# IllyaArtemchuk/Harmonies-Alphazero

Measured on AMD Instinct MI355X. Metric: self-play env-steps/sec + games/sec @4096 boards, 1/2/4/8 GPUs; bit-exact vs CPU, higher is better.
Workload: dtype u64; 1 GPU; config2: 4096 concurrent boards/GPU, reset + rule-driven play to game end (legal mask, step, chance draws, final scoring); one step = 256 hz_play launches of 4096 boards; boards_per_gpu=4096, parallelism=shard1

## Files before the change

harmonies-alphazero_amd/csrc/hz_device.hpp:

```cpp
#pragma once
#include <hip/hip_runtime.h>
#include <stdint.h>

namespace hz {

constexpr int kCells = 23;
constexpr uint32_t kAll23 = (1u << 23) - 1;
constexpr int kActions = 143;
enum { WATER = 0, PLANT = 1, WOOD = 2, STONE = 3, BUILDING = 4, FIELD = 5 };
enum { PH_CHOOSE = 0, PH_P1 = 1, PH_P2 = 2, PH_P3 = 3, PH_OVER = 4 };
enum {
  ST_OK = 0, ST_BAD_PILE = 1, ST_BAD_FORMAT = 2, ST_NOT_IN_HAND = 3, ST_ILLEGAL_STACK = 4,
  ST_BAD_PHASE = 5, ST_BAD_ACTION = 6, ST_NOOP = 7
};

__host__ __device__ constexpr int initial_count(int t) {
  return t == WATER ? 23 : t == PLANT ? 19 : t == WOOD ? 21 : t == STONE ? 23 : t == BUILDING ? 15 : 19;
}

struct State {
  uint64_t pl[4];
  uint64_t piles;
  uint64_t misc;
};

__device__ __forceinline__ int hand_tile(uint64_t m, int j) { return (int)((m >> (3 * j)) & 7); }
__device__ __forceinline__ int hand_n(uint64_t m) { return (int)((m >> 9) & 3); }
__device__ __forceinline__ int bag_n(uint64_t m, int t) { return (int)((m >> (11 + 5 * t)) & 31); }
__device__ __forceinline__ int player_of(uint64_t m) { return (int)((m >> 41) & 1); }
__device__ __forceinline__ int phase_of(uint64_t m) { return (int)((m >> 42) & 7); }
__device__ __forceinline__ int over_flag(uint64_t m) { return (int)((m >> 45) & 1); }
__device__ __forceinline__ int winner_code(uint64_t m) { return (int)((m >> 46) & 3); }
__device__ __forceinline__ int score_of(uint64_t m, int p) { return (int)((m >> (48 + 8 * p)) & 255); }
__device__ __forceinline__ int npiles_of(uint64_t piles) { return (int)((piles >> 45) & 7); }
__device__ __forceinline__ int pile_tile(uint64_t piles, int i, int j) { return (int)((piles >> (9 * i + 3 * j)) & 7); }
// ... 323 lines not shown
    if (pos >= kMT) { pos = 0; tw = 0; }
    while (tw < kMT && tw < pos + W) tw += twist_block_vec(w, tw);
    left = tw - pos < W ? tw - pos : W;
    const int a = pos & ~3, sh = pos & 3;
    uint32_t f[W + 4];
#pragma unroll
    for (int k = 0; k < W / 4 + 1; k++) {
      const int o = a + 4 * k <= kMT - 4 ? a + 4 * k : kMT - 4;
      const uint4 v = *(const uint4*)(w + o);
      f[4 * k] = v.x; f[4 * k + 1] = v.y; f[4 * k + 2] = v.z; f[4 * k + 3] = v.w;
    }
#pragma unroll
    for (int j = 0; j < W; j++) q[j] = sh == 0 ? f[j] : sh == 1 ? f[j + 1] : sh == 2 ? f[j + 2] : f[j + 3];
  }

  __device__ __forceinline__ uint32_t next() {
    fresh = false;
    if (left > 0) {
      const uint32_t v = q[0];
#pragma unroll
      for (int j = 0; j + 1 < W; j++) q[j] = q[j + 1];
      left--;
      pos++;
      return temper(v);
    }
    if (pos >= kMT) { pos = 0; tw = 0; }
    if (pos >= tw) tw += twist_block(w, 1, tw);
    return temper(w[pos++]);
  }
};
using WinMT12 = WinGMT<12>;

constexpr int kLdsStride = 65;
extern __shared__ uint32_t hz_lds[];

struct LdsMT {
  int lane, pos, tw;
  __device__ __forceinline__ LdsMT(int l, int cursor) : lane(l), pos(cursor & 0xFFFF), tw(cursor >> 16) {}
  __device__ __forceinline__ int cursor() const { return pos | (tw << 16); }
  __device__ __forceinline__ uint32_t* w() const { return hz_lds + lane; }

  __device__ __forceinline__ void prefetch() {
    if (pos >= kMT) { pos = 0; tw = 0; }
    while (tw < kMT && tw < pos + 24) tw += twist_block(w(), kLdsStride, tw);
  }

  __device__ __forceinline__ uint32_t word(int i) const {
    return temper(hz_lds[(i < kMT ? i : kMT - 1) * kLdsStride + lane]);
  }

  __device__ __forceinline__ uint32_t next() {
    if (pos >= kMT) { pos = 0; tw = 0; }
    if (pos >= tw) tw += twist_block(w(), kLdsStride, tw);
    return word(pos++);
  }

  __device__ __forceinline__ void normalize() {
    if (pos >= kMT) return;
    while (tw < kMT) tw += twist_block(w(), kLdsStride, tw);
  }

  __device__ __forceinline__ void twist_ahead(int target) {
    if (pos >= kMT) { pos = 0; tw = 0; }
    while (tw < target) tw += twist_block(w(), kLdsStride, tw);
  }
};

constexpr int kAheadTwist = 224;
constexpr int kMTAhead = 0 | (kAheadTwist << 16);

struct InitGen { uint32_t v[kMT]; };
constexpr InitGen make_init_gen() {
  InitGen g{};
  uint32_t x = 19650218u;
  g.v[0] = x;
  for (int i = 1; i < kMT; i++) {
    x = 1812433253u * (x ^ (x >> 30)) + (uint32_t)i;
    g.v[i] = x;
  }
  return g;
}
__constant__ InitGen kInitGen = make_init_gen();

struct NoProgress {
  __device__ __forceinline__ void operator()(int) const {}
};
template <class Ptr, class Prog = NoProgress>
__device__ __forceinline__ void mt_seed(Ptr w, int stride, uint64_t seed, Prog prog = Prog()) {
  uint32_t key0 = (uint32_t)seed, key1 = (uint32_t)(seed >> 32);
  uint32_t kA = key0, kB = key1 ? key1 + 1u : key0;
  uint32_t prev = 19650218u;
  uint32_t iv[8];
#pragma unroll
  for (int u = 0; u < 8; u++) iv[u] = kInitGen.v[1 + u];
  for (int g = 1; g < kMT - 7; g += 8) {
    uint32_t nx[8];
#pragma unroll
    for (int u = 0; u < 8; u++) nx[u] = kInitGen.v[g + 8 + u < kMT ? g + 8 + u : kMT - 1];
#pragma unroll
    for (int u = 0; u < 8; u++) {
      uint32_t v = (iv[u] ^ ((prev ^ (prev >> 30)) * 1664525U)) + ((u & 1) ? kB : kA);
      w[(g + u) * stride] = v;
      prev = v;
    }
#pragma unroll
    for (int u = 0; u < 8; u++) iv[u] = nx[u];
  }
#pragma unroll
  for (int u = 0; u < 7; u++) {
    uint32_t v = (iv[u] ^ ((prev ^ (prev >> 30)) * 1664525U)) + ((u & 1) ? kB : kA);
    w[(617 + u) * stride] = v;
    prev = v;
  }
  uint32_t m1 = w[1 * stride];
// ... 171 lines not shown

template <class M>
__device__ __forceinline__ uint32_t randbelow(M& m, uint32_t n) {
  if (!n) return 0;
  int k = 32 - __clz(n);
  uint32_t r = m.next() >> (32 - k);
  while (r >= n) r = m.next() >> (32 - k);
  return r;
}

template <class M>
__device__ __forceinline__ void sample3_serial(M& m, uint32_t n, int k, uint32_t j[3], int got) {
  if (n <= 21) {
    for (int i = got; i < k; i++) j[i] = randbelow(m, n - (uint32_t)i);
  } else {
    for (int i = got; i < k; i++) {
      uint32_t v;
      bool dup;
      do {
        v = randbelow(m, n);
        dup = (i > 0 && j[0] == v) || (i > 1 && j[1] == v);
      } while (dup);
      j[i] = v;
    }
  }
}

template <class M>
__device__ __forceinline__ void sample3_raw(M& m, uint32_t n, int k, uint32_t j[3]) {
  sample3_serial(m, n, k, j, 0);
}

typedef __attribute__((address_space(3))) const volatile uint32_t LdsVolatileWord;
template <bool Clamp>
__device__ __forceinline__ uint32_t scan_word(const LdsMT& m, int t) {
  LdsVolatileWord* lds = (LdsVolatileWord*)hz_lds;
  if (Clamp) {
    int i = m.pos + t < kMT ? m.pos + t : kMT - 1;
    return lds[i * kLdsStride + m.lane];
  }
  return lds[(m.pos + t) * kLdsStride + m.lane];
}

__device__ __forceinline__ uint32_t sgpr_const(uint32_t v) {
  uint32_t r;
  asm volatile("s_mov_b32 %0, %1" : "=s"(r) : "i"(v));
  return r;
}
struct TemperMasks {
  uint32_t b, c;
  __device__ __forceinline__ TemperMasks() : b(sgpr_const(0x9d2c5680u)), c(sgpr_const(0xefc60000u)) {}
};
__device__ __forceinline__ uint32_t and_xor(uint32_t x, uint32_t m, uint32_t y) {
  uint32_t r;
  asm("v_bitop3_b32 %0, %1, %2, %3 bitop3:0x6a" : "=v"(r) : "v"(x), "s"(m), "v"(y));
  return r;
}
__device__ __forceinline__ uint32_t temper_top14(uint32_t y, const TemperMasks& k) {
  y ^= y >> 11;
  y = and_xor(y << 7, k.b, y);
  y = and_xor(y << 15, k.c, y);
  return y;
}
__device__ __forceinline__ uint32_t temper_top14(uint32_t y) {
  y ^= y >> 11;
  y ^= (y << 7) & 0x9d2c5680u;
  y ^= (y << 15) & 0xefc60000u;
  return y;
}

template <bool Clamp, bool Pool>
__device__ __forceinline__ int scan3(LdsMT& m, uint32_t n, uint32_t& p0, uint32_t& p1, uint32_t& p2) {
  int avail = m.tw - m.pos;
  uint32_t lim = n;
  int sh = __clz(n);
  uint32_t j0 = 0xffffffffu, j1 = 0xffffffffu, j2 = 0xffffffffu;
  int got = 0, used = 0;
  TemperMasks tk;
  uint32_t w[4], nx[4];
#pragma unroll
  for (int u = 0; u < 4; u++) nx[u] = scan_word<Clamp>(m, u);
#pragma unroll
  for (int seg = 0; seg < 6; seg++) {
#pragma unroll
    for (int u = 0; u < 4; u++) w[u] = nx[u];
    if (seg < 5) {
#pragma unroll
      for (int u = 0; u < 4; u++) nx[u] = scan_word<Clamp>(m, 4 * seg + 4 + u);
    }
#pragma unroll
    for (int u = 0; u < 4; u++) {
      int t = 4 * seg + u;
      bool live = got < 3;
      if (Clamp) live = live && t < avail;
      uint32_t v = temper_top14(w[u], tk) >> sh;
      bool ok = live && v < lim;
      if (!Pool) ok = ok && v != j0 && v != j1;
      j2 = ok ? j1 : j2;
      j1 = ok ? j0 : j1;
      j0 = ok ? v : j0;
      got += ok ? 1 : 0;
      used += live ? 1 : 0;
      if (Pool) {
        lim -= ok ? 1u : 0u;
        sh = __clz(lim);
      }
    }
    if (__all(got >= 3)) break;
  }
  m.pos += used;
  p0 = got == 3 ? j2 : got == 2 ? j1 : j0;
  p1 = got == 3 ? j1 : j0;
  p2 = j0;
  return got;
}

__device__ __forceinline__ void sample3_raw(LdsMT& m, uint32_t n, int k, uint32_t j[3]) {
  if (k != 3) {
    sample3_serial(m, n, k, j, 0);
    return;
  }
  uint32_t j0, j1, j2;
  int got;
  bool far = __any(m.pos > kMT - 24);
  if (__all(n > 21)) {
    if (far) got = scan3<true, false>(m, n, j0, j1, j2);
    else got = scan3<false, false>(m, n, j0, j1, j2);
  } else if (__all(n <= 21)) {
    if (far) got = scan3<true, true>(m, n, j0, j1, j2);
    else got = scan3<false, true>(m, n, j0, j1, j2);
  } else {
    if (n > 21) got = scan3<true, false>(m, n, j0, j1, j2);
    else got = scan3<true, true>(m, n, j0, j1, j2);
  }
  j[0] = j0; j[1] = j1; j[2] = j2;
  if (got < k) sample3_serial(m, n, k, j, got);
}

struct WinMT : LdsMT {
  int lim;
  __device__ __forceinline__ WinMT(int l, int cursor, int rows) : LdsMT(l, cursor), lim(rows) {}
  __device__ __forceinline__ void prefetch() {}
  __device__ __forceinline__ uint32_t next() {
    const int i = pos++;
    return i < lim ? temper(hz_lds[i * kLdsStride + lane]) : 0x9E3779B9u * (uint32_t)(i + 1);
  }
};
__device__ __forceinline__ void sample3_raw(WinMT& m, uint32_t n, int k, uint32_t j[3]) {
  if (k != 3) {
    sample3_serial(m, n, k, j, 0);
    return;
  }
  uint32_t j0, j1, j2;
  int got;
  LdsMT& lm = m;
  if (__all(n > 21)) got = scan3<false, false>(lm, n, j0, j1, j2);
  else if (__all(n <= 21)) got = scan3<false, true>(lm, n, j0, j1, j2);
  else if (n > 21) got = scan3<false, false>(lm, n, j0, j1, j2);
  else got = scan3<false, true>(lm, n, j0, j1, j2);
  j[0] = j0; j[1] = j1; j[2] = j2;
  if (got < k) sample3_serial(m, n, k, j, got);
}

template <class M>
__device__ __forceinline__ int draw_pile(uint64_t misc, M& m, uint32_t& pile9) {
  int cnt[6];
#pragma unroll
  for (int t = 0; t < 6; t++) cnt[t] = bag_n(misc, t);
  uint32_t n = 0;
#pragma unroll
  for (int t = 0; t < 6; t++) n += (uint32_t)cnt[t];
  pile9 = 0x1FF;
  if (!n) return 0;
  int k = n < 3 ? (int)n : 3;
  uint32_t j[3] = {0, 0, 0};
  sample3_raw(m, n, k, j);
  uint32_t idx[3];
  if (n <= 21) {
    uint32_t mp0 = 0xffffffffu, mp1 = 0xffffffffu, mv0 = 0, mv1 = 0;
#pragma unroll
    for (int i = 0; i < 3; i++) {
      uint32_t ji = j[i], last = n - (uint32_t)i - 1;
      uint32_t vj = ji, vl = last;
      if (i > 0 && mp0 == ji) vj = mv0;
      if (i > 1 && mp1 == ji) vj = mv1;
      if (i > 0 && mp0 == last) vl = mv0;
      if (i > 1 && mp1 == last) vl = mv1;
      idx[i] = vj;
      if (i == 0) { mp0 = ji; mv0 = vl; }
      if (i == 1) { mp1 = ji; mv1 = vl; }
    }
  } else {
// ... 645 lines not shown
```

harmonies-alphazero_amd/csrc/hz_env.hip:

```cpp
#include <hip/hip_runtime.h>

#include <cstdio>
#include <cstdlib>
#include <cstring>

#include "../../include/hz_abi.h"
#include "hz_device.hpp"
#include "hz_encode.hpp"
#include "hz_host.hpp"

using namespace hz;
using namespace hz_host;

struct P2Draw {
  int32_t *tag;
  int32_t *k;
  uint64_t *q;
  uint64_t *bag;
  int32_t *c;
};
struct P2Mid {
  int32_t *tag;
  uint64_t *st;
  uint64_t *q;
// ... 1244 lines not shown
    ply[b] = g_ply;
    seed[b] = sd;
#if defined(HZ_DIAG) && !defined(HZ_DIAG_ROLES_ONLY)
    if (g_stamps) {
      uint64_t *o = g_stamps + (size_t)b * 16;
      o[8] = acc8; o[9] = acc9; o[10] = acc10; o[11] = acc11; o[12] = acc12; o[13] = acc13;
    }
#endif
    if (games_done) games_done[b] = games;
    if (steps_done) steps_done[b] = steps;
    if (ep_final) ep_final[b] = episode[b];
    uint64_t lm = __ballot(lds_used);
    if (lane == 0) s_lds_mask = lm;
  }
  if (w0 && !act && lane == 0 && actmask == 0) s_lds_mask = 0;
  __syncthreads();
  uint64_t lds_mask = s_lds_mask & actmask;
  if (lds_mask) stage_mt(g, nb, tid, lds_mask, false);
#ifdef HZ_DIAG
  if (g_stamps && threadIdx.x < 64 && act) g_stamps[(size_t)b * 16 + 5] = __builtin_amdgcn_s_memtime() - role_t0;
#endif
}

#ifndef HZ_P2_ST_WT
#define HZ_P2_ST_WT 0
#endif
#ifndef HZ_P2_AUX
#define HZ_P2_AUX 16
#endif
constexpr int kP2Win = 96;
constexpr int kP2WinRows = kP2Win + 24;
#ifndef HZ_P2_DCUT
#if HZ_P2_NDRAW == 5
#define HZ_P2_DCUT 0, 5, 10, 14, 18
#elif HZ_P2_NDRAW == 4
#define HZ_P2_DCUT 0, 7, 13, 18
#endif
#endif
constexpr int kP2DCut[kP2Draw] = {HZ_P2_DCUT};
constexpr int kP2StageDraws = 7;
#ifndef HZ_P2_PCUT
#if HZ_P2_NPLAY == 5
#define HZ_P2_PCUT 16, 32, 48, 64
#elif HZ_P2_NPLAY == 4
#define HZ_P2_PCUT 24, 40, 56
#endif
#endif
constexpr int kP2PCut[kP2Play - 1] = {HZ_P2_PCUT};
enum { kWvP1 = 8, kWvHash = 9, kWvPlay = 10, kWvIdle = 15 };
#ifndef HZ_P2_WAVES
#if HZ_P2_NDRAW == 5 && HZ_P2_NPLAY == 5
#define HZ_P2_WAVES 0, 1, 4, 9, 2, 3, 8, 10
#elif HZ_P2_NDRAW == 5
#define HZ_P2_WAVES 0, 1, 4, 9, 2, 3, 8, 15
#elif HZ_P2_NPLAY == 5
#define HZ_P2_WAVES 0, 1, 8, 9, 2, 3, 10, 15
#else
#define HZ_P2_WAVES 0, 1, 8, 9, 2, 3, 15, 15
#endif
#endif
constexpr int kP2Wave[8] = {HZ_P2_WAVES};
constexpr int p2_wave_count(int code) {
  int c = 0;
  for (int k = 0; k < 8; k++) c += kP2Wave[k] == code;
  return c;
}
constexpr bool p2_waves_ok() {
  for (int d = 0; d < 5; d++)
    if (p2_wave_count(d) != (d < kP2Draw ? 1 : 0)) return false;
  return p2_wave_count(kWvP1) == 1 && p2_wave_count(kWvHash) == 1 && p2_wave_count(kWvPlay) == (kP2Play == 5 ? 1 : 0);
}
static_assert(p2_waves_ok(), "HZ_P2_WAVES: every stage outside the seed and play blocks on exactly one wave");
constexpr int kP2MinPlies = 96;
#ifdef HZ_DIAG
constexpr int kP2Stamps = 48;
#define P2_PHASE(slot, t0)                                                                                       \
  do {                                                                                                           \
    __builtin_amdgcn_sched_barrier(0);                                                                           \
    if (g_stamps && b < a.n) g_stamps[(size_t)b * kP2Stamps + (slot)] = __builtin_amdgcn_s_memtime() - (t0); \
    __builtin_amdgcn_sched_barrier(0);                                                                           \
  } while (0)
#else
#define P2_PHASE(slot, t0) \
  do {                     \
  } while (0)
#endif
static_assert(4 * kP2WinRows * kLdsStride * 4 <= (int)kResetLds, "a window per wave of a draw block");

struct P2Args {
  uint64_t *st;
  uint32_t *mt;
  int32_t *pos, *ply, *episode;
  uint64_t *seed;
  int n, max_plies, draws;
  int cut[kP2Play - 1];
  int dcut[kP2Draw + 1];
  uint64_t seed_base;
  long nrow;
  int32_t *games_done, *steps_done, *mt_src;
  const int32_t *ep_in;
  int32_t *ep_out;
  uint32_t *s_mt[kP2Stages];
  int32_t *s_tag[kP2Stages];
  int32_t *s_cur[kP2Stages];
  int s_idx_last;
  uint32_t *p1h_w;
  const uint32_t *p1h_r;
  int32_t *p1t_w;
  const int32_t *p1t_r;
  uint32_t *p2h_w;
  const uint32_t *p2h_r;
  uint32_t *p3h_w;
  const uint32_t *p3h_r;
  P2Draw x_w[kP2Draw - 1], x_r[kP2Draw - 1];
  P2Draw pl_w, pl_r[kP2Play];
  P2Mid m_w[kP2Play - 1], m_r[kP2Play - 1];
  uint32_t *h_w;
  const uint32_t *h_r[kP2Play];
  int32_t *ht_w;
  const int32_t *ht_r[kP2Play];
// ... 121 lines not shown
    v = kMT + 1;
  }
  return v;
}
__device__ __forceinline__ void p2_publish(int *flag, int v) {
  asm volatile("" ::: "memory");
  __hip_atomic_store(flag, v, __ATOMIC_RELAXED, __HIP_MEMORY_SCOPE_WORKGROUP);
}
__device__ __forceinline__ __amdgpu_buffer_rsrc_t p2_slot_rsrc(uint32_t *slot, int b0, size_t nr) {
  const uint64_t base = (uint64_t)(slot + b0);
  uint32_t lo = __builtin_amdgcn_readfirstlane((uint32_t)base), hi = __builtin_amdgcn_readfirstlane((uint32_t)(base >> 32));
  const int bytes = __builtin_amdgcn_readfirstlane((int)((size_t)kMT * nr * 4 - (size_t)b0 * 4));
  return __builtin_amdgcn_make_buffer_rsrc((void *)(((uint64_t)hi << 32) | lo), 0, bytes, 0x00020000);
}
#ifndef HZ_P2_LDNT
#define HZ_P2_LDNT 0
#endif
__device__ __forceinline__ uint4 p2_ld4(const uint32_t *p) {
  if constexpr (HZ_P2_LDNT) {
    typedef uint32_t v4u __attribute__((ext_vector_type(4)));
    const v4u v = __builtin_nontemporal_load((const v4u *)p);
    return make_uint4(v[0], v[1], v[2], v[3]);
  }
  return *reinterpret_cast<const uint4 *>(p);
}
template <class T>
__device__ __forceinline__ void p2_st(T *p, T v) {
  if constexpr (HZ_P2_AUX == 16 && HZ_P2_ST_WT) __hip_atomic_store(p, v, __ATOMIC_RELAXED, __HIP_MEMORY_SCOPE_AGENT);
  else *p = v;
}
__device__ __forceinline__ uint32_t p1_step(uint32_t t, uint32_t q, bool odd, uint32_t kA, uint32_t kB) {
  return (t ^ ((q ^ (q >> 30)) * 1664525U)) + (odd ? kA : kB);
}
__device__ __forceinline__ int p2_tab(int i) { return i < kMT ? i : kMT - 1; }
__device__ __forceinline__ uint32_t p1_row1(uint32_t kA, uint32_t kB) {
  return p1_step(kInitGen.v[1], 19650218u, true, kA, kB);
}
__device__ __forceinline__ void p2_keys(uint64_t seed, uint32_t &kA, uint32_t &kB) {
  const uint32_t key0 = (uint32_t)seed, key1 = (uint32_t)(seed >> 32);
  kA = key0;
  kB = key1 ? key1 + 1u : key0;
}

__device__ __forceinline__ void p2_p1(const P2Args &a, int b) {
  const int e = a.ep_in[b] + kP2Last;
  uint32_t kA, kB;
  p2_keys(episode_seed(a.seed_base, b, e), kA, kB);
  uint32_t prev = 19650218u;
  uint32_t iv[8];
#pragma unroll
  for (int u = 0; u < 8; u++) iv[u] = kInitGen.v[1 + u];
#pragma unroll 1
  for (int g = 1; g < 617; g += 8) {
    uint32_t nx[8];
#pragma unroll
    for (int u = 0; u < 8; u++) nx[u] = kInitGen.v[p2_tab(g + 8 + u)];
    __builtin_amdgcn_sched_barrier(0);
#pragma unroll
    for (int u = 0; u < 8; u++) prev = p1_step(iv[u], prev, !(u & 1), kA, kB);
    __builtin_amdgcn_sched_barrier(0);
#pragma unroll
    for (int u = 0; u < 8; u++) iv[u] = nx[u];
  }
#pragma unroll
  for (int u = 0; u < 7; u++) prev = p1_step(iv[u], prev, !(u & 1), kA, kB);
  a.p1h_w[b] = p1_step(p1_row1(kA, kB), prev, false, kA, kB);
  a.p1t_w[b] = e * 8 + 2;
}

constexpr int kP2aEnd = 209, kP2bEnd = 417;
constexpr int kTwKeep = 397;
struct P2Ahead {
  uint32_t cur[8];
  uint32_t iv[8];
  uint32_t last;
};
template <int G>
__device__ __forceinline__ void p2_ahead_init(P2Ahead &h, uint32_t q, uint32_t kA, uint32_t kB) {
#pragma unroll
  for (int u = 0; u < 8; u++) {
    q = p1_step(kInitGen.v[p2_tab(G + u)], q, (G + u) & 1, kA, kB);
    h.cur[u] = q;
  }
#pragma unroll
  for (int u = 0; u < 8; u++) h.iv[u] = kInitGen.v[p2_tab(G + 8 + u)];
  h.last = q;
}
__device__ __forceinline__ uint32_t twist_part(uint32_t cur, uint32_t next) {
  const uint32_t y = (cur & 0x80000000U) | (next & 0x7fffffffU);
  return (y >> 1) ^ ((y & 1U) ? 0x9908b0dfU : 0U);
}
enum { kP2Final = 0, kP2Keep = 1, kP2Part = 2 };
template <int G0, int G1, int Mode>
__device__ __forceinline__ void p2_span(int lane, __amdgpu_buffer_rsrc_t rs, int row_bytes, uint32_t &prev, P2Ahead &h,
                                        uint32_t kA, uint32_t kB, int *prog) {
  constexpr bool KeepLds = Mode == kP2Keep;
  static_assert((G1 - G0) % 8 == 0, "groups of eight");
  uint32_t *l = hz_lds + lane;
  constexpr int S = kLdsStride;
#pragma unroll 2
  for (int g = G0; g < G1; g += 8) {
    uint32_t ivn[8], nx[8];
#pragma unroll
    for (int u = 0; u < 8; u++) ivn[u] = kInitGen.v[p2_tab(g + 16 + u)];
    const uint32_t kneg = __builtin_amdgcn_readfirstlane(0u - (uint32_t)g);
    const int soff = __builtin_amdgcn_readfirstlane((Mode == kP2Part ? g - 1 : g) * row_bytes);
    uint32_t q = h.cur[7];
#pragma unroll
    for (int u = 0; u < 8; u++) {
      const uint32_t p = (prev ^ (prev >> 30)) * 1566083941U;
      uint32_t v;
      asm("v_xad_u32 %0, %1, %2, %3" : "=v"(v) : "v"(p), "v"(h.cur[u]), "s"(kneg - (uint32_t)u));
      __builtin_amdgcn_raw_buffer_store_b32(Mode == kP2Part ? twist_part(prev, v) : v, rs, lane * 4,
                                            soff + u * row_bytes, HZ_P2_AUX);
      if (KeepLds) l[(g + u) * S] = v;
      prev = v;
      q = p1_step(h.iv[u], q, (G0 + u) & 1, kA, kB);
      nx[u] = q;
    }
    if (KeepLds) p2_publish(prog, g + 8);
    h.last = h.cur[7];
#pragma unroll
    for (int u = 0; u < 8; u++) {
      h.cur[u] = nx[u];
      h.iv[u] = ivn[u];
    }
  }
}
template <int G, int G1, int Mode>
__device__ __forceinline__ void p2_tail(int lane, __amdgpu_buffer_rsrc_t rs, int row_bytes, uint32_t &prev, P2Ahead &h) {
  static_assert(G1 - G >= 1 && G1 - G <= 8, "within the group ahead");
#pragma unroll
  for (int i = G; i < G1; i++) {
    const uint32_t v = (h.cur[i - G] ^ ((prev ^ (prev >> 30)) * 1566083941U)) - (uint32_t)i;
    if (Mode == kP2Part) __builtin_amdgcn_raw_buffer_store_b32(twist_part(prev, v), rs, lane * 4, (i - 1) * row_bytes, HZ_P2_AUX);
    else __builtin_amdgcn_raw_buffer_store_b32(v, rs, lane * 4, i * row_bytes, HZ_P2_AUX);
    if (Mode == kP2Keep) hz_lds[i * kLdsStride + lane] = v;
    prev = v;
  }
  h.last = h.cur[G1 - G - 1];
}

template <int K>
__device__ __forceinline__ void p2_third(const P2Args &a, int b0, int lane, int e, bool ok, int *s_prog) {
  const int b = b0 + lane;
  const bool act = b < a.n;
  const size_t nr = (size_t)a.nrow;
  if (K == 0 && act && !ok) a.s_tag[1][b] = -1;
  if (!__any(ok)) {
    if (K == 2) p2_publish(s_prog, kMT + 1);
    return;
  }
  uint32_t *slot = a.s_mt[1 + K];
  uint32_t kA, kB;
  p2_keys(episode_seed(a.seed_base, b, e), kA, kB);
  uint32_t prev, first1, row2, q;
  if (K == 0) {
    first1 = act ? a.p1h_r[b] : 0u;
    prev = first1;
    q = p1_row1(kA, kB);
  } else {
    const uint32_t *h = K == 1 ? a.p2h_r : a.p3h_r;
    prev = act ? h[b] : 0u;
    first1 = act ? h[nr + b] : 0u;
    row2 = act ? h[2 * nr + b] : 0u;
    q = act ? h[3 * nr + b] : 0u;
  }
  const __amdgpu_buffer_rsrc_t rs = p2_slot_rsrc(slot, b0, nr);
  const int row_bytes = (int)(nr * 4);
  P2Ahead h;
  if constexpr (K == 0) {
    q = p1_step(kInitGen.v[2], q, false, kA, kB);
    row2 = (q ^ ((prev ^ (prev >> 30)) * 1566083941U)) - 2U;
    prev = row2;
    p2_ahead_init<3>(h, q, kA, kB);
    constexpr int G = 3 + 8 * ((kP2aEnd - 3) / 8);
    p2_span<3, G, kP2Part>(lane, rs, row_bytes, prev, h, kA, kB, s_prog);
    p2_tail<G, kP2aEnd, kP2Part>(lane, rs, row_bytes, prev, h);
  } else if constexpr (K == 1) {
    static_assert(kAheadTwist + 1 - kP2aEnd == 16, "P2b's part steps: two groups");
    p2_ahead_init<kP2aEnd>(h, q, kA, kB);
    p2_span<kP2aEnd, kAheadTwist + 1, kP2Part>(lane, rs, row_bytes, prev, h, kA, kB, s_prog);
    __builtin_amdgcn_raw_buffer_store_b32(prev, rs, lane * 4, kAheadTwist * row_bytes, HZ_P2_AUX);
    p2_span<kAheadTwist + 1, kP2bEnd, kP2Final>(lane, rs, row_bytes, prev, h, kA, kB, s_prog);
  } else {
    const uint32_t f0 = act ? slot[(size_t)397 * nr + b] : 0u, f1 = act ? slot[(size_t)398 * nr + b] : 0u;
    p2_ahead_init<kP2bEnd>(h, q, kA, kB);
    constexpr int G = kP2bEnd + 8 * ((kMT - kP2bEnd) / 8);
    p2_span<kP2bEnd, G, kP2Keep>(lane, rs, row_bytes, prev, h, kA, kB, s_prog);
    p2_tail<G, kMT, kP2Keep>(lane, rs, row_bytes, prev, h);
    p2_publish(s_prog, kMT);
    const uint32_t row1 = (first1 ^ ((prev ^ (prev >> 30)) * 1566083941U)) - 1U;
    __builtin_amdgcn_raw_buffer_store_b32(f0 ^ twist_part(0x80000000u, row1), rs, lane * 4, 0, HZ_P2_AUX);
    __builtin_amdgcn_raw_buffer_store_b32(f1 ^ twist_part(row1, row2), rs, lane * 4, row_bytes, HZ_P2_AUX);
  }
  if (K < 2) {
    if (ok) {
      uint32_t *ho = K == 0 ? a.p2h_w : a.p3h_w;
      ho[b] = prev;
      ho[nr + b] = first1;
      ho[2 * nr + b] = row2;
      ho[3 * nr + b] = h.last;
      a.s_tag[1 + K][b] = e * 8 + 3 + K;
    }
  } else if (ok) {
    a.s_tag[3][b] = e * 8 + 5;
  }
}

constexpr int kTwIters = kAheadTwist / 4;
constexpr int kTwHbm = (kP2bEnd - 397 + 3) / 4;
__device__ __forceinline__ uint4 xor4(const uint4 &a, const uint4 &b) {
  return make_uint4(a.x ^ b.x, a.y ^ b.y, a.z ^ b.z, a.w ^ b.w);
}
__device__ __forceinline__ void p2_twist(const P2Args &a, int b0, int lane, bool any, int *s_prog) {
  if (!any) return;
  const size_t nr = (size_t)a.nrow;
  uint32_t *slot = a.s_mt[3];
  const int grp = lane >> 4, c4 = (lane & 15) * 4;
  uint32_t *col = slot + b0 + c4;
  auto row = [&](int r) { return p2_ld4(col + (size_t)r * nr); };
  const __amdgpu_buffer_rsrc_t rs = p2_slot_rsrc(slot, b0, nr);
  const int row_bytes = __builtin_amdgcn_readfirstlane((int)(nr * 4));
// ... 43 lines not shown
  const bool act = b < a.n;
  if (tid == 0) s_prog = 0;
  const int k = w < 3 ? w : 2;
  const int e = act ? a.ep_in[b] + kP2Last - 1 - k : 0;
  const bool ok = act && (k == 0 ? a.p1t_r[b] : a.s_tag[1 + k][b]) == e * 8 + 2 + k;
  __syncthreads();
  if (w == 0) p2_third<0>(a, b0, lane, e, ok, &s_prog);
  else if (w == 1) p2_third<1>(a, b0, lane, e, ok, &s_prog);
  else if (w == 2) p2_third<2>(a, b0, lane, e, ok, &s_prog);
  else p2_twist(a, b0, lane, __any(ok), &s_prog);
}

__device__ __forceinline__ int wave_min_i(int v) {
#pragma unroll
  for (int o = 32; o > 0; o >>= 1) v = min(v, __shfl_xor(v, o));
  return v;
}
__device__ __forceinline__ void p2_draw_stage(const P2Args &a, int b0, int lane, int stage, int base) {
  const int b = b0 + lane;
#ifdef HZ_DIAG
  const uint64_t t0 = __builtin_amdgcn_s_memtime();
#endif
  const bool act = b < a.n;
  const size_t nr = (size_t)a.nrow;
  const int d0 = a.dcut[stage], d1 = stage == kP2Draw - 1 ? a.draws : min(a.draws, a.dcut[stage + 1]);
  const int e = act ? a.ep_in[b] + kP2Last - kP2SDraw - stage : 0;
  const uint32_t *slot = a.s_mt[kP2SDraw + stage];
  int32_t *cur = a.s_cur[kP2SDraw + stage] + b;
  const P2Draw &in = a.x_r[stage > 0 ? stage - 1 : 0];
  const P2Draw &out = stage == kP2Draw - 1 ? a.pl_w : a.x_w[stage < kP2Draw - 1 ? stage : 0];
  bool ok = act && a.s_tag[kP2SDraw + stage][b] == e * 8 + 5;
  int k0 = 0, c0 = kMTAhead;
  uint64_t bag = initial_bag(), q[kAheadWords] = {0, 0, 0, 0};
  if (stage > 0 && act) {
    const int itag = in.tag[b];
    k0 = in.k[b];
    c0 = in.c[b];
    bag = in.bag[b];
#pragma unroll
    for (int i = 0; i < kAheadWords; i++) q[i] = in.q[(size_t)i * nr + b];
    ok = ok && itag == e * 8 + stage;
  }
  const bool draws = ok && k0 >= d0 && d0 < d1;
  const int r0 = wave_min_i(draws ? (c0 & 0xFFFF) : kAheadTwist) & ~3;
  if (r0 < kAheadTwist) {
    constexpr int U = kP2Win / 4;
    const int c4 = (lane & 15) * 4;
    uint4 v[U];
#pragma unroll
    for (int u = 0; u < U; u++) {
      const int r = r0 + 4 * u + (lane >> 4);
      v[u] = p2_ld4(slot + (size_t)r * nr + b0 + c4);
    }
#pragma unroll
    for (int u = 0; u < U; u++) {
      uint32_t *dd = hz_lds + base + (4 * u + (lane >> 4)) * kLdsStride + c4;
      dd[0] = v[u].x;
      dd[1] = v[u].y;
      dd[2] = v[u].z;
      dd[3] = v[u].w;
    }
  }
  P2_PHASE(28 + stage, t0);
  if (!act) return;
  if (!ok) {
    out.tag[b] = -1;
    return;
  }
  if (stage == 0) cur[0] = kMTAhead;
  int k = k0, cc = c0;
  if (draws) {
    const int lim = min(r0 + kP2Win, kAheadTwist);
    StreamDraw<WinMT> d{WinMT(base - r0 * kLdsStride + lane, c0, lim)};
#pragma unroll 1
    for (int i = d0; i < d1; i++) {
      if (d.m.pos >= lim) break;
      const uint32_t p9 = d(bag);
      if (d.m.pos > lim) break;
      apply_pile_fast(bag, p9);
      const int bit = 9 * i, wd = bit >> 6, off = bit & 63;
      const uint64_t lo9 = (uint64_t)p9 << off, hi9 = off > 55 ? (uint64_t)p9 >> (64 - off) : 0ull;
      q[0] |= wd == 0 ? lo9 : 0ull;
      q[1] |= wd == 1 ? lo9 : wd == 0 ? hi9 : 0ull;
      q[2] |= wd == 2 ? lo9 : wd == 1 ? hi9 : 0ull;
      q[3] |= wd == 3 ? lo9 : wd == 2 ? hi9 : 0ull;
      cc = d.m.cursor();
      p2_st(&cur[(size_t)(i + 1) * nr], cc);
      k = i + 1;
    }
  }
  p2_st(&out.k[b], k);
  p2_st(&out.c[b], cc);
  p2_st(&out.bag[b], bag);
#pragma unroll
  for (int i = 0; i < kAheadWords; i++) p2_st(&out.q[(size_t)i * nr + b], q[i]);
  p2_st(&out.tag[b], e * 8 + stage + 1);
}

__device__ __forceinline__ void p2_hashes(const P2Args &a, int b) {
  const size_t nr = (size_t)a.nrow;
  const int e = a.ep_in[b] + kP2Last - (kP2SPlay - 1);
  const uint64_t rk = rule_key(episode_seed(a.seed_base, b, e));
#pragma unroll 1
  for (int j = 0; j < kRulePlies; j++) p2_st(&a.h_w[(size_t)j * nr + b], rule_h32(rk, j));
  a.ht_w[b] = e;
}

__device__ __forceinline__ void p2_draw(const P2Args &a, int blk, int code) {
  const int tid = threadIdx.x, lane = tid & 63, w = tid >> 6;
  const int b0 = blk * kBlock;
  if (code < kP2Draw) {
    p2_draw_stage(a, b0, lane, code, w * kP2WinRows * kLdsStride);
  } else if (code == kWvP1 && b0 + lane < a.n) {
    p2_p1(a, b0 + lane);
  } else if (code == kWvHash && b0 + lane < a.n) {
    p2_hashes(a, b0 + lane);
  }
}

__device__ __forceinline__ void p2_mid_put(const P2Mid &m, size_t nr, int b, const State &s, const PlayDraw2 &d, int g,
                                           int e) {
#pragma unroll
  for (int k = 0; k < 4; k++) p2_st(&m.st[(size_t)k * nr + b], s.pl[k]);
  p2_st(&m.st[4 * nr + b], s.piles);
  p2_st(&m.st[5 * nr + b], s.misc);
  p2_st(&m.q[b], d.q0);
  p2_st(&m.q[nr + b], d.q1);
  p2_st(&m.q[2 * nr + b], d.q2);
  p2_st(&m.q[3 * nr + b], d.q3);
  p2_st(&m.i[b], d.d);
  p2_st(&m.i[nr + b], g);
  p2_st(&m.i[2 * nr + b], d.fell ? d.gm.cursor() : -1);
  p2_st(&m.tag[b], e);
}
__device__ __forceinline__ PlayDraw2 p2_mid_get(const P2Mid &m, size_t nr, int b, State &s, int &g, int nd,
                                               uint32_t *slot, const int32_t *cur) {
#pragma unroll
  for (int k = 0; k < 4; k++) s.pl[k] = m.st[(size_t)k * nr + b];
  s.piles = m.st[4 * nr + b];
  s.misc = m.st[5 * nr + b];
  const int d = m.i[b], fc = m.i[2 * nr + b];
  g = m.i[nr + b];
  return PlayDraw2{m.q[b], m.q[nr + b], m.q[2 * nr + b], m.q[3 * nr + b], d, nd, fc >= 0,
                   MTR(slot, (int)nr, fc >= 0 ? fc : 0), cur + (size_t)nd * nr};
}
// ... 781 lines not shown
```

Before: 21.66 billion env-steps/s.

## Vectorize MT init-table scalar loads, pad LDS window stride, rebalance draw stages

Pads the constant MT init table so row 1 sits on a 64-byte boundary and the read-ahead needs no clamping. The P1 seeding loop can then use double-buffered s_load_dwordx8 scalar loads, and the P2 spans read the table through a constant-address-space pointer. The draw window in LDS gets a stride of 68 so rows are 16-byte aligned and can be written with uint4 stores. Stage 0 issues its window load before reading the previous stage's inputs. It also moves the P2b/P2c split point and the draw-stage cut points, and uses v_bfi in twist_part. The risks are scalar-load hazards from the inline asm, a larger LDS footprint and retuned stage balance.

```diff
diff --git a/harmonies-alphazero_amd/csrc/hz_device.hpp b/harmonies-alphazero_amd/csrc/hz_device.hpp
--- a/harmonies-alphazero_amd/csrc/hz_device.hpp
+++ b/harmonies-alphazero_amd/csrc/hz_device.hpp
@@ -1,6 +1,8 @@
 #pragma once
 #include <hip/hip_runtime.h>
 #include <stdint.h>
+
+#include "hz_initgen.hpp"
 
 namespace hz {
 
@@ -390,7 +392,7 @@
 using WinMT12 = WinGMT<12>;
 
 constexpr int kLdsStride = 65;
-extern __shared__ uint32_t hz_lds[];
+extern __shared__ __attribute__((aligned(16))) uint32_t hz_lds[];
 
 struct LdsMT {
   int lane, pos, tw;
@@ -427,17 +429,7 @@
 constexpr int kAheadTwist = 224;
 constexpr int kMTAhead = 0 | (kAheadTwist << 16);
 
-struct InitGen { uint32_t v[kMT]; };
-constexpr InitGen make_init_gen() {
-  InitGen g{};
-  uint32_t x = 19650218u;
-  g.v[0] = x;
-  for (int i = 1; i < kMT; i++) {
-    x = 1812433253u * (x ^ (x >> 30)) + (uint32_t)i;
-    g.v[i] = x;
-  }
-  return g;
-}
+static_assert(kInitGenRows == kMT, "the table's rows");
 __constant__ InitGen kInitGen = make_init_gen();
 
 struct NoProgress {
@@ -675,14 +667,14 @@
 }
 
 typedef __attribute__((address_space(3))) const volatile uint32_t LdsVolatileWord;
-template <bool Clamp>
+template <bool Clamp, int Stride = kLdsStride>
 __device__ __forceinline__ uint32_t scan_word(const LdsMT& m, int t) {
   LdsVolatileWord* lds = (LdsVolatileWord*)hz_lds;
   if (Clamp) {
     int i = m.pos + t < kMT ? m.pos + t : kMT - 1;
-    return lds[i * kLdsStride + m.lane];
-  }
-  return lds[(m.pos + t) * kLdsStride + m.lane];
+    return lds[i * Stride + m.lane];
+  }
+  return lds[(m.pos + t) * Stride + m.lane];
 }
 
 __device__ __forceinline__ uint32_t sgpr_const(uint32_t v) {
@@ -712,7 +704,7 @@
   return y;
 }
 
-template <bool Clamp, bool Pool>
+template <bool Clamp, bool Pool, int Stride = kLdsStride>
 __device__ __forceinline__ int scan3(LdsMT& m, uint32_t n, uint32_t& p0, uint32_t& p1, uint32_t& p2) {
   int avail = m.tw - m.pos;
   uint32_t lim = n;
@@ -722,14 +714,14 @@
   TemperMasks tk;
   uint32_t w[4], nx[4];
 #pragma unroll
-  for (int u = 0; u < 4; u++) nx[u] = scan_word<Clamp>(m, u);
+  for (int u = 0; u < 4; u++) nx[u] = scan_word<Clamp, Stride>(m, u);
 #pragma unroll
   for (int seg = 0; seg < 6; seg++) {
 #pragma unroll
     for (int u = 0; u < 4; u++) w[u] = nx[u];
     if (seg < 5) {
 #pragma unroll
-      for (int u = 0; u < 4; u++) nx[u] = scan_word<Clamp>(m, 4 * seg + 4 + u);
+      for (int u = 0; u < 4; u++) nx[u] = scan_word<Clamp, Stride>(m, 4 * seg + 4 + u);
     }
 #pragma unroll
     for (int u = 0; u < 4; u++) {
@@ -780,13 +772,14 @@
   if (got < k) sample3_serial(m, n, k, j, got);
 }
 
+constexpr int kWinStride = 68;
 struct WinMT : LdsMT {
   int lim;
   __device__ __forceinline__ WinMT(int l, int cursor, int rows) : LdsMT(l, cursor), lim(rows) {}
   __device__ __forceinline__ void prefetch() {}
   __device__ __forceinline__ uint32_t next() {
     const int i = pos++;
-    return i < lim ? temper(hz_lds[i * kLdsStride + lane]) : 0x9E3779B9u * (uint32_t)(i + 1);
+    return i < lim ? temper(hz_lds[i * kWinStride + lane]) : 0x9E3779B9u * (uint32_t)(i + 1);
   }
 };
 __device__ __forceinline__ void sample3_raw(WinMT& m, uint32_t n, int k, uint32_t j[3]) {
@@ -797,10 +790,10 @@
   uint32_t j0, j1, j2;
   int got;
   LdsMT& lm = m;
-  if (__all(n > 21)) got = scan3<false, false>(lm, n, j0, j1, j2);
-  else if (__all(n <= 21)) got = scan3<false, true>(lm, n, j0, j1, j2);
-  else if (n > 21) got = scan3<false, false>(lm, n, j0, j1, j2);
-  else got = scan3<false, true>(lm, n, j0, j1, j2);
+  if (__all(n > 21)) got = scan3<false, false, kWinStride>(lm, n, j0, j1, j2);
+  else if (__all(n <= 21)) got = scan3<false, true, kWinStride>(lm, n, j0, j1, j2);
+  else if (n > 21) got = scan3<false, false, kWinStride>(lm, n, j0, j1, j2);
+  else got = scan3<false, true, kWinStride>(lm, n, j0, j1, j2);
   j[0] = j0; j[1] = j1; j[2] = j2;
   if (got < k) sample3_serial(m, n, k, j, got);
 }
diff --git a/harmonies-alphazero_amd/csrc/hz_env.hip b/harmonies-alphazero_amd/csrc/hz_env.hip
--- a/harmonies-alphazero_amd/csrc/hz_env.hip
+++ b/harmonies-alphazero_amd/csrc/hz_env.hip
@@ -1300,7 +1300,7 @@
 constexpr int kP2WinRows = kP2Win + 24;
 #ifndef HZ_P2_DCUT
 #if HZ_P2_NDRAW == 5
-#define HZ_P2_DCUT 0, 5, 10, 14, 18
+#define HZ_P2_DCUT 0, 6, 11, 15, 19
 #elif HZ_P2_NDRAW == 4
 #define HZ_P2_DCUT 0, 7, 13, 18
 #endif
@@ -1353,7 +1353,7 @@
   do {                     \
   } while (0)
 #endif
-static_assert(4 * kP2WinRows * kLdsStride * 4 <= (int)kResetLds, "a window per wave of a draw block");
+static_assert(4 * kP2WinRows * kWinStride * 4 <= (int)kResetLds, "a window per wave of a draw block");
 
 struct P2Args {
   uint64_t *st;
@@ -1541,7 +1541,6 @@
 __device__ __forceinline__ uint32_t p1_step(uint32_t t, uint32_t q, bool odd, uint32_t kA, uint32_t kB) {
   return (t ^ ((q ^ (q >> 30)) * 1664525U)) + (odd ? kA : kB);
 }
-__device__ __forceinline__ int p2_tab(int i) { return i < kMT ? i : kMT - 1; }
 __device__ __forceinline__ uint32_t p1_row1(uint32_t kA, uint32_t kB) {
   return p1_step(kInitGen.v[1], 19650218u, true, kA, kB);
 }
@@ -1551,83 +1550,132 @@
   kB = key1 ? key1 + 1u : key0;
 }
 
+typedef uint32_t u32x8 __attribute__((ext_vector_type(8)));
+template <int Imm>
+__device__ __forceinline__ u32x8 p1_load8(const uint32_t *tab, uint32_t off) {
+  u32x8 t;
+  asm volatile("s_load_dwordx8 %0, %1, %2 offset:%3" : "=&s"(t) : "s"(tab), "s"(off), "n"(Imm));
+  return t;
+}
+__device__ __forceinline__ void p1_arrived(u32x8 &t) { asm volatile("s_waitcnt lgkmcnt(0)" : "+s"(t)); }
+__device__ __forceinline__ uint32_t p1_steps8(const u32x8 &t, uint32_t prev, uint32_t kA, uint32_t kB) {
+#pragma unroll
+  for (int u = 0; u < 8; u++) prev = p1_step(t[u], prev, !(u & 1), kA, kB);
+  return prev;
+}
 __device__ __forceinline__ void p2_p1(const P2Args &a, int b) {
   const int e = a.ep_in[b] + kP2Last;
   uint32_t kA, kB;
   p2_keys(episode_seed(a.seed_base, b, e), kA, kB);
   uint32_t prev = 19650218u;
-  uint32_t iv[8];
-#pragma unroll
-  for (int u = 0; u < 8; u++) iv[u] = kInitGen.v[1 + u];
+  const uint32_t *tab = kInitGen.v + 1;
+  static_assert(38 * 16 + 1 == 609 && 617 + 8 <= kMT + kInitGenPad, "the last group's read (rows 617-624) within the table's padding");
+  u32x8 ta = p1_load8<0>(tab, 0), tb;
+  p1_arrived(ta);
 #pragma unroll 1
-  for (int g = 1; g < 617; g += 8) {
-    uint32_t nx[8];
-#pragma unroll
-    for (int u = 0; u < 8; u++) nx[u] = kInitGen.v[p2_tab(g + 8 + u)];
+  for (uint32_t off = 0; off < 38 * 64; off += 64) {
+    tb = p1_load8<32>(tab, off);
     __builtin_amdgcn_sched_barrier(0);
-#pragma unroll
-    for (int u = 0; u < 8; u++) prev = p1_step(iv[u], prev, !(u & 1), kA, kB);
+    prev = p1_steps8(ta, prev, kA, kB);
     __builtin_amdgcn_sched_barrier(0);
-#pragma unroll
-    for (int u = 0; u < 8; u++) iv[u] = nx[u];
-  }
-#pragma unroll
-  for (int u = 0; u < 7; u++) prev = p1_step(iv[u], prev, !(u & 1), kA, kB);
+    p1_arrived(tb);
+    ta = p1_load8<64>(tab, off);
+    __builtin_amdgcn_sched_barrier(0);
+    prev = p1_steps8(tb, prev, kA, kB);
+    __builtin_amdgcn_sched_barrier(0);
+    p1_arrived(ta);
+  }
+  tb = p1_load8<0>(tab, (617 - 1) * 4);
+  prev = p1_steps8(ta, prev, kA, kB);
+  p1_arrived(tb);
+#pragma unroll
+  for (int u = 0; u < 7; u++) prev = p1_step(tb[u], prev, !(u & 1), kA, kB);
   a.p1h_w[b] = p1_step(p1_row1(kA, kB), prev, false, kA, kB);
   a.p1t_w[b] = e * 8 + 2;
 }
 
-constexpr int kP2aEnd = 209, kP2bEnd = 417;
-constexpr int kTwKeep = 397;
+#ifndef HZ_P2_BEND
+#define HZ_P2_BEND 433
+#endif
+constexpr int kP2aEnd = 209, kP2bEnd = HZ_P2_BEND;
+static_assert(kP2bEnd > 399 && kP2bEnd + 64 < kMT && (kP2bEnd - kAheadTwist - 1) % 8 == 0, "P2b's final steps in groups of eight; rows 397, 398 P2b's");
 struct P2Ahead {
   uint32_t cur[8];
   uint32_t iv[8];
   uint32_t last;
 };
+typedef __attribute__((address_space(4))) const uint32_t ConstWord;
+__device__ __forceinline__ ConstWord *p2_table() {
+  ConstWord *t = (ConstWord *)kInitGen.v;
+  asm volatile("" : "+s"(t));
+  return t;
+}
 template <int G>
-__device__ __forceinline__ void p2_ahead_init(P2Ahead &h, uint32_t q, uint32_t kA, uint32_t kB) {
+__device__ __forceinline__ void p2_ahead_init(ConstWord *tab, P2Ahead &h, uint32_t q, uint32_t kA, uint32_t kB) {
 #pragma unroll
   for (int u = 0; u < 8; u++) {
-    q = p1_step(kInitGen.v[p2_tab(G + u)], q, (G + u) & 1, kA, kB);
+    q = p1_step(tab[G + u], q, (G + u) & 1, kA, kB);
     h.cur[u] = q;
   }
 #pragma unroll
-  for (int u = 0; u < 8; u++) h.iv[u] = kInitGen.v[p2_tab(G + 8 + u)];
+  for (int u = 0; u < 8; u++) h.iv[u] = tab[G + 8 + u];
   h.last = q;
 }
 __device__ __forceinline__ uint32_t twist_part(uint32_t cur, uint32_t next) {
-  const uint32_t y = (cur & 0x80000000U) | (next & 0x7fffffffU);
-  return (y >> 1) ^ ((y & 1U) ? 0x9908b0dfU : 0U);
+  uint32_t y;
+  asm("v_bfi_b32 %0, %1, %2, %3" : "=v"(y) : "s"(0x7fffffffU), "v"(next), "v"(cur));
+  return (y >> 1) ^ ((next & 1U) ? 0x9908b0dfU : 0U);
 }
 enum { kP2Final = 0, kP2Keep = 1, kP2Part = 2 };
+typedef __attribute__((address_space(3))) uint32_t LdsWord;
+struct P2Out {
+  __amdgpu_buffer_rsrc_t rs;
+  int row_bytes;
+  int vo[8];
+  uint32_t lds;
+  __device__ __forceinline__ P2Out(__amdgpu_buffer_rsrc_t r, int rb, int lane) : rs(r), row_bytes(rb) {
+#pragma unroll
+    for (int u = 0; u < 8; u++) {
+      vo[u] = lane * 4 + u * rb;
+      asm volatile("" : "+v"(vo[u]));
+    }
+    lds = (uint32_t)(uintptr_t)(LdsWord *)(hz_lds + lane);
+  }
+  __device__ __forceinline__ void put(uint32_t v, int soff, int u) const {
+    __builtin_amdgcn_raw_buffer_store_b32(v, rs, vo[u], soff, HZ_P2_AUX);
+  }
+};
 template <int G0, int G1, int Mode>
-__device__ __forceinline__ void p2_span(int lane, __amdgpu_buffer_rsrc_t rs, int row_bytes, uint32_t &prev, P2Ahead &h,
-                                        uint32_t kA, uint32_t kB, int *prog) {
+__device__ __forceinline__ void p2_span(ConstWord *tab, const P2Out &o, uint32_t &prev, P2Ahead &h, uint32_t kA, uint32_t kB, int *prog) {
   constexpr bool KeepLds = Mode == kP2Keep;
   static_assert((G1 - G0) % 8 == 0, "groups of eight");
-  uint32_t *l = hz_lds + lane;
+  static_assert(G1 + 15 < kMT + kInitGenPad, "the table's read-ahead within its padding");
   constexpr int S = kLdsStride;
+  uint32_t lg = o.lds + G0 * S * 4;
 #pragma unroll 2
   for (int g = G0; g < G1; g += 8) {
     uint32_t ivn[8], nx[8];
 #pragma unroll
-    for (int u = 0; u < 8; u++) ivn[u] = kInitGen.v[p2_tab(g + 16 + u)];
+    for (int u = 0; u < 8; u++) ivn[u] = tab[g + 16 + u];
     const uint32_t kneg = __builtin_amdgcn_readfirstlane(0u - (uint32_t)g);
-    const int soff = __builtin_amdgcn_readfirstlane((Mode == kP2Part ? g - 1 : g) * row_bytes);
+    const int soff = __builtin_amdgcn_readfirstlane((Mode == kP2Part ? g - 1 : g) * o.row_bytes);
+    if (KeepLds) asm volatile("" : "+v"(lg));
     uint32_t q = h.cur[7];
 #pragma unroll
     for (int u = 0; u < 8; u++) {
       const uint32_t p = (prev ^ (prev >> 30)) * 1566083941U;
       uint32_t v;
       asm("v_xad_u32 %0, %1, %2, %3" : "=v"(v) : "v"(p), "v"(h.cur[u]), "s"(kneg - (uint32_t)u));
-      __builtin_amdgcn_raw_buffer_store_b32(Mode == kP2Part ? twist_part(prev, v) : v, rs, lane * 4,
-                                            soff + u * row_bytes, HZ_P2_AUX);
-      if (KeepLds) l[(g + u) * S] = v;
+      o.put(Mode == kP2Part ? twist_part(prev, v) : v, soff, u);
+      if (KeepLds) *(LdsWord *)(uintptr_t)(lg + u * S * 4) = v;
       prev = v;
       q = p1_step(h.iv[u], q, (G0 + u) & 1, kA, kB);
       nx[u] = q;
     }
-    if (KeepLds) p2_publish(prog, g + 8);
+    if (KeepLds) {
+      p2_publish(prog, g + 8);
+      lg += 8 * S * 4;
+    }
     h.last = h.cur[7];
 #pragma unroll
     for (int u = 0; u < 8; u++) {
@@ -1637,13 +1685,13 @@
   }
 }
 template <int G, int G1, int Mode>
-__device__ __forceinline__ void p2_tail(int lane, __amdgpu_buffer_rsrc_t rs, int row_bytes, uint32_t &prev, P2Ahead &h) {
+__device__ __forceinline__ void p2_tail(const P2Out &o, int lane, uint32_t &prev, P2Ahead &h) {
   static_assert(G1 - G >= 1 && G1 - G <= 8, "within the group ahead");
+  const int soff = __builtin_amdgcn_readfirstlane((Mode == kP2Part ? G - 1 : G) * o.row_bytes);
 #pragma unroll
   for (int i = G; i < G1; i++) {
     const uint32_t v = (h.cur[i - G] ^ ((prev ^ (prev >> 30)) * 1566083941U)) - (uint32_t)i;
-    if (Mode == kP2Part) __builtin_amdgcn_raw_buffer_store_b32(twist_part(prev, v), rs, lane * 4, (i - 1) * row_bytes, HZ_P2_AUX);
-    else __builtin_amdgcn_raw_buffer_store_b32(v, rs, lane * 4, i * row_bytes, HZ_P2_AUX);
+    o.put(Mode == kP2Part ? twist_part(prev, v) : v, soff, i - G);
     if (Mode == kP2Keep) hz_lds[i * kLdsStride + lane] = v;
     prev = v;
   }
@@ -1676,28 +1724,30 @@
     q = act ? h[3 * nr + b] : 0u;
   }
   const __amdgpu_buffer_rsrc_t rs = p2_slot_rsrc(slot, b0, nr);
-  const int row_bytes = (int)(nr * 4);
+  const int row_bytes = __builtin_amdgcn_readfirstlane((int)(nr * 4));
+  const P2Out o(rs, row_bytes, lane);
+  ConstWord *tab = p2_table();
   P2Ahead h;
   if constexpr (K == 0) {
     q = p1_step(kInitGen.v[2], q, false, kA, kB);
     row2 = (q ^ ((prev ^ (prev >> 30)) * 1566083941U)) - 2U;
     prev = row2;
-    p2_ahead_init<3>(h, q, kA, kB);
+    p2_ahead_init<3>(tab, h, q, kA, kB);
     constexpr int G = 3 + 8 * ((kP2aEnd - 3) / 8);
-    p2_span<3, G, kP2Part>(lane, rs, row_bytes, prev, h, kA, kB, s_prog);
-    p2_tail<G, kP2aEnd, kP2Part>(lane, rs, row_bytes, prev, h);
+    p2_span<3, G, kP2Part>(tab, o, prev, h, kA, kB, s_prog);
+    p2_tail<G, kP2aEnd, kP2Part>(o, lane, prev, h);
   } else if constexpr (K == 1) {
     static_assert(kAheadTwist + 1 - kP2aEnd == 16, "P2b's part steps: two groups");
-    p2_ahead_init<kP2aEnd>(h, q, kA, kB);
-    p2_span<kP2aEnd, kAheadTwist + 1, kP2Part>(lane, rs, row_bytes, prev, h, kA, kB, s_prog);
+    p2_ahead_init<kP2aEnd>(tab, h, q, kA, kB);
+    p2_span<kP2aEnd, kAheadTwist + 1, kP2Part>(tab, o, prev, h, kA, kB, s_prog);
     __builtin_amdgcn_raw_buffer_store_b32(prev, rs, lane * 4, kAheadTwist * row_bytes, HZ_P2_AUX);
-    p2_span<kAheadTwist + 1, kP2bEnd, kP2Final>(lane, rs, row_bytes, prev, h, kA, kB, s_prog);
+    p2_span<kAheadTwist + 1, kP2bEnd, kP2Final>(tab, o, prev, h, kA, kB, s_prog);
   } else {
     const uint32_t f0 = act ? slot[(size_t)397 * nr + b] : 0u, f1 = act ? slot[(size_t)398 * nr + b] : 0u;
-    p2_ahead_init<kP2bEnd>(h, q, kA, kB);
+    p2_ahead_init<kP2bEnd>(tab, h, q, kA, kB);
     constexpr int G = kP2bEnd + 8 * ((kMT - kP2bEnd) / 8);
-    p2_span<kP2bEnd, G, kP2Keep>(lane, rs, row_bytes, prev, h, kA, kB, s_prog);
-    p2_tail<G, kMT, kP2Keep>(lane, rs, row_bytes, prev, h);
+    p2_span<kP2bEnd, G, kP2Keep>(tab, o, prev, h, kA, kB, s_prog);
+    p2_tail<G, kMT, kP2Keep>(o, lane, prev, h);
     p2_publish(s_prog, kMT);
     const uint32_t row1 = (first1 ^ ((prev ^ (prev >> 30)) * 1566083941U)) - 1U;
     __builtin_amdgcn_raw_buffer_store_b32(f0 ^ twist_part(0x80000000u, row1), rs, lane * 4, 0, HZ_P2_AUX);
@@ -1807,6 +1857,22 @@
   bool ok = act && a.s_tag[kP2SDraw + stage][b] == e * 8 + 5;
   int k0 = 0, c0 = kMTAhead;
   uint64_t bag = initial_bag(), q[kAheadWords] = {0, 0, 0, 0};
+  constexpr int U = kP2Win / 4;
+  const int c4 = (lane & 15) * 4;
+  uint4 v[U];
+  auto win_load = [&](int r0) {
+#pragma unroll
+    for (int u = 0; u < U; u++) {
+      const int r = r0 + 4 * u + (lane >> 4);
+      v[u] = p2_ld4(slot + (size_t)r * nr + b0 + c4);
+    }
+  };
+  auto win_store = [&]() {
+#pragma unroll
+    for (int u = 0; u < U; u++)
+      *reinterpret_cast<uint4 *>(hz_lds + base + (4 * u + (lane >> 4)) * kWinStride + c4) = v[u];
+  };
+  if (stage == 0) win_load(0);
   if (stage > 0 && act) {
     const int itag = in.tag[b];
     k0 = in.k[b];
@@ -1819,22 +1885,8 @@
   const bool draws = ok && k0 >= d0 && d0 < d1;
   const int r0 = wave_min_i(draws ? (c0 & 0xFFFF) : kAheadTwist) & ~3;
   if (r0 < kAheadTwist) {
-    constexpr int U = kP2Win / 4;
-    const int c4 = (lane & 15) * 4;
-    uint4 v[U];
-#pragma unroll
-    for (int u = 0; u < U; u++) {
-      const int r = r0 + 4 * u + (lane >> 4);
-      v[u] = p2_ld4(slot + (size_t)r * nr + b0 + c4);
-    }
-#pragma unroll
-    for (int u = 0; u < U; u++) {
-      uint32_t *dd = hz_lds + base + (4 * u + (lane >> 4)) * kLdsStride + c4;
-      dd[0] = v[u].x;
-      dd[1] = v[u].y;
-      dd[2] = v[u].z;
-      dd[3] = v[u].w;
-    }
+    if (stage > 0) win_load(r0);
+    win_store();
   }
   P2_PHASE(28 + stage, t0);
   if (!act) return;
@@ -1846,7 +1898,7 @@
   int k = k0, cc = c0;
   if (draws) {
     const int lim = min(r0 + kP2Win, kAheadTwist);
-    StreamDraw<WinMT> d{WinMT(base - r0 * kLdsStride + lane, c0, lim)};
+    StreamDraw<WinMT> d{WinMT(base - r0 * kWinStride + lane, c0, lim)};
 #pragma unroll 1
     for (int i = d0; i < d1; i++) {
       if (d.m.pos >= lim) break;
@@ -1885,7 +1937,7 @@
   const int tid = threadIdx.x, lane = tid & 63, w = tid >> 6;
   const int b0 = blk * kBlock;
   if (code < kP2Draw) {
-    p2_draw_stage(a, b0, lane, code, w * kP2WinRows * kLdsStride);
+    p2_draw_stage(a, b0, lane, code, w * kP2WinRows * kWinStride);
   } else if (code == kWvP1 && b0 + lane < a.n) {
     p2_p1(a, b0 + lane);
   } else if (code == kWvHash && b0 + lane < a.n) {
diff --git a/harmonies-alphazero_amd/csrc/hz_initgen.hpp b/harmonies-alphazero_amd/csrc/hz_initgen.hpp
--- /dev/null
+++ b/harmonies-alphazero_amd/csrc/hz_initgen.hpp
@@ -0,0 +1,25 @@
+#pragma once
+#include <stddef.h>
+#include <stdint.h>
+
+namespace hz {
+
+constexpr int kInitGenRows = 624, kInitGenPad = 16;
+struct InitGen {
+  alignas(64) uint32_t lead[15];
+  uint32_t v[kInitGenRows + kInitGenPad];
+};
+constexpr InitGen make_init_gen() {
+  InitGen g{};
+  uint32_t x = 19650218u;
+  g.v[0] = x;
+  for (int i = 1; i < kInitGenRows; i++) {
+    x = 1812433253u * (x ^ (x >> 30)) + (uint32_t)i;
+    g.v[i] = x;
+  }
+  for (int i = kInitGenRows; i < kInitGenRows + kInitGenPad; i++) g.v[i] = x;
+  return g;
+}
+static_assert(offsetof(InitGen, v) % 64 == 60, "row 1 of the table on a 64-byte boundary");
+
+}
```

New measurement: 22.91 billion env-steps/s, median of 6. +5.8%, better.
